# wangrui2025/GDKVM

Hardware: AMD Instinct MI355X
Metric: frames/sec (GDKVM forward + argmax mask), EchoNet 112x112x32 clips (higher is better)
Workload: dtype bf16; 1 GPU; BASELINE.json configs[1]: EchoNet-Dynamic 112x112x32 bf16 inference, batch=16 per GPU; clips_per_gpu=16, frames_per_clip=32, image=112x112, heads=1, key_dim=64, rule=delta_sequential, world_size=1, ranks_seen=1

## Files before the change

gdkvm_amd/csrc/conv_dispatch.hip:

```cpp
#include "gdkvm_common.hpp"

int gdkvm_conv3x3_c64_launch(const void* x, const void* w, const float* bias, const void* residual, void* y, int N, int H, int W,
                             int relu, int packed, hipStream_t st);
int gdkvm_conv3x3_tile_launch(const void* x, const void* x2, int C1, const void* w, const float* bias, const void* residual, void* y,
                              int N, int C, int H, int W, int K, int relu, int variant, int packed, hipStream_t st);
int gdkvm_conv_igemm_launch(const void* x, const void* wpacked, const float* bias, const void* residual, void* y,
                            int N, int C, int H, int W, int K, int R, int S, int stride, int pad, int relu,
                            const void* w2packed, const float* bias2, void* y2, hipStream_t st);

extern "C" int gdkvm_conv_bias_act(const void* x, const void* w, const float* bias, const void* residual, void* y,
                                   int N, int C, int H, int W, int K, int R, int S, int stride, int pad, int relu, int kernel,
                                   int io_dtype, void* stream)
{
    if (io_dtype != GDKVM_BF16) return gdkvm_fail(GDKVM_ERR_DTYPE, "conv_bias_act: only bf16 is implemented");
    if (N < 0 || C <= 0 || H <= 0 || W <= 0 || K <= 0 || R <= 0 || S <= 0 || stride <= 0 || pad < 0 || C % 8 || K % 8
        || H + 2 * pad < R || W + 2 * pad < S)
        return gdkvm_fail(GDKVM_ERR_SHAPE, "conv_bias_act: N=%d C=%d H=%d W=%d K=%d %dx%d stride %d pad %d (C, K multiples of 8)",
                          N, C, H, W, K, R, S, stride, pad);
    const bool packed = kernel & GDKVM_CONV_PACKED_WEIGHTS;
    kernel &= ~GDKVM_CONV_PACKED_WEIGHTS;
    if (kernel != 0 && (kernel < 4 || kernel > 11)) return gdkvm_fail(GDKVM_ERR_ARG, "conv_bias_act: kernel=%d (0 = by shape, 4, 5, 6..8, 9, 10, 11)", kernel);
    if (kernel == 9) {
        if (!packed) return gdkvm_fail(GDKVM_ERR_ARG, "conv_bias_act: kernel 9 reads the gdkvm_conv_igemm_pack_weights copy of the weights (flag %d)", GDKVM_CONV_PACKED_WEIGHTS);
        if (C % 32 || K % 128) return gdkvm_fail(GDKVM_ERR_SHAPE, "conv_bias_act: kernel 9 needs C a multiple of 32 and K of 128 (C=%d K=%d)", C, K);
        if (N == 0) return GDKVM_OK;
        if (!x || !w || !bias || !y) return gdkvm_fail(GDKVM_ERR_ARG, "conv_bias_act: null pointer");
        if (!gdkvm_aligned16(x) || !gdkvm_aligned16(w) || !gdkvm_aligned16(y) || !gdkvm_aligned16(bias) || (residual && !gdkvm_aligned16(residual)))
            return gdkvm_fail(GDKVM_ERR_ARG, "conv_bias_act: pointers must be 16-byte aligned");
        if (int rc = gdkvm_check_device()) return rc;
        if (gdkvm_conv_igemm_launch(x, w, bias, residual, y, N, C, H, W, K, R, S, stride, pad, relu, nullptr, nullptr, nullptr, static_cast<hipStream_t>(stream)))
            return gdkvm_fail(GDKVM_ERR_SHAPE, "conv_bias_act: N=%d C=%d H=%d W=%d K=%d %dx%d stride %d pad %d is too large for 32-bit offsets", N, C, H, W, K, R, S, stride, pad);
        GDKVM_LAUNCH_CHECK("conv_igemm_kernel");
        return GDKVM_OK;
    }
    if (packed && (C % 64 || K % 16))
        return gdkvm_fail(GDKVM_ERR_ARG, "conv_bias_act: packed weights need C a multiple of 64 and K of 16 (C=%d K=%d)", C, K);
    if (!(R == 3 && S == 3 && stride == 1 && pad == 1))
        return gdkvm_fail(GDKVM_ERR_SHAPE, "conv_bias_act: %dx%d stride %d pad %d is not served by the 3x3 / 1 / 1 kernels: kernel 9 (the "
                                           "implicit-GEMM kernel, packed weights) or the framework convolution + gdkvm_bias_act", R, S, stride, pad);
    if (N == 0) return GDKVM_OK;
    if (!x || !w || !bias || !y) return gdkvm_fail(GDKVM_ERR_ARG, "conv_bias_act: null pointer");
    if (!gdkvm_aligned16(x) || !gdkvm_aligned16(w) || !gdkvm_aligned16(y) || !gdkvm_aligned16(bias) || (residual && !gdkvm_aligned16(residual)))
        return gdkvm_fail(GDKVM_ERR_ARG, "conv_bias_act: pointers must be 16-byte aligned");
    if ((size_t)N * H * W * C >= (1ull << 31) || (size_t)N * H * W * K >= (1ull << 31))
        return gdkvm_fail(GDKVM_ERR_SHAPE, "conv_bias_act: tensor too large for 32-bit offsets");
    if (int rc = gdkvm_check_device()) return rc;
    hipStream_t st = static_cast<hipStream_t>(stream);
    const bool c64 = C == 64 && K == 64;
    if (kernel == 4 && !c64) return gdkvm_fail(GDKVM_ERR_SHAPE, "conv_bias_act: kernel 4 serves 64 -> 64 channels only (C=%d K=%d)", C, K);
    if (kernel == 4 || (kernel == 0 && c64)) {
        if (gdkvm_conv3x3_c64_launch(x, w, bias, residual, y, N, H, W, relu, packed ? 1 : 0, st)) return gdkvm_fail(GDKVM_ERR_SHAPE, "conv_bias_act: too many tiles");
        GDKVM_LAUNCH_CHECK("conv3x3_c64_kernel");
        return GDKVM_OK;
    }
    if (gdkvm_conv3x3_tile_launch(x, nullptr, 0, w, bias, residual, y, N, C, H, W, K, relu, kernel >= 10 ? kernel - 6 : (kernel >= 6 ? kernel - 5 : 0), packed ? 1 : 0, st))
        return gdkvm_fail(GDKVM_ERR_SHAPE, "conv_bias_act: C=%d K=%d %dx%d is not served by the hand-written kernels (C a multiple of 64, K of "
                                           "16, rows of at most 64 pixels): use the framework convolution + gdkvm_bias_act", C, K, H, W);
    GDKVM_LAUNCH_CHECK("conv3x3_tile_kernel");
    return GDKVM_OK;
}

extern "C" int gdkvm_conv_cat_bias_act(const void* x1, const void* x2, const void* w, const float* bias, const void* residual, void* y,
                                       int N, int C1, int C2, int H, int W, int K, int relu, int kernel, int io_dtype, void* stream)
{
    if (io_dtype != GDKVM_BF16) return gdkvm_fail(GDKVM_ERR_DTYPE, "conv_cat_bias_act: only bf16 is implemented");
    const bool packed = kernel & GDKVM_CONV_PACKED_WEIGHTS;
    kernel &= ~GDKVM_CONV_PACKED_WEIGHTS;
    if (kernel != 0 && (kernel < 5 || kernel > 11 || kernel == 9)) return gdkvm_fail(GDKVM_ERR_ARG, "conv_cat_bias_act: kernel=%d (0, 5..8, 10, 11)", kernel);
    if (N < 0 || C1 <= 0 || C2 <= 0 || C1 % 64 || C2 % 64 || H <= 0 || W <= 0 || K <= 0 || K % 16)
        return gdkvm_fail(GDKVM_ERR_SHAPE, "conv_cat_bias_act: N=%d C1=%d C2=%d H=%d W=%d K=%d (C1, C2 multiples of 64, K of 16)", N, C1, C2, H, W, K);
    if (N == 0) return GDKVM_OK;
    if (!x1 || !x2 || !w || !bias || !y) return gdkvm_fail(GDKVM_ERR_ARG, "conv_cat_bias_act: null pointer");
    if (!gdkvm_aligned16(x1) || !gdkvm_aligned16(x2) || !gdkvm_aligned16(w) || !gdkvm_aligned16(y) || !gdkvm_aligned16(bias) || (residual && !gdkvm_aligned16(residual)))
        return gdkvm_fail(GDKVM_ERR_ARG, "conv_cat_bias_act: pointers must be 16-byte aligned");
    if ((size_t)N * H * W * (C1 + C2) >= (1ull << 31) || (size_t)N * H * W * K >= (1ull << 31))
        return gdkvm_fail(GDKVM_ERR_SHAPE, "conv_cat_bias_act: tensor too large for 32-bit offsets");
    if (int rc = gdkvm_check_device()) return rc;
    if (gdkvm_conv3x3_tile_launch(x1, x2, C1, w, bias, residual, y, N, C1 + C2, H, W, K, relu, kernel >= 10 ? kernel - 6 : (kernel >= 6 ? kernel - 5 : 0), packed ? 1 : 0,
                                  static_cast<hipStream_t>(stream)))
        return gdkvm_fail(GDKVM_ERR_SHAPE, "conv_cat_bias_act: %dx%d is not served (rows of at most 64 pixels)", H, W);
    GDKVM_LAUNCH_CHECK("conv3x3_tile_kernel");
    return GDKVM_OK;
}

extern "C" int gdkvm_conv_down_bias_act(const void* x, const void* w, const float* bias, void* y, int relu,
                                        const void* w_down, const float* bias_down, void* y_down,
                                        int N, int C, int H, int W, int K, int R, int S, int stride, int pad, int io_dtype, void* stream)
{
    if (io_dtype != GDKVM_BF16) return gdkvm_fail(GDKVM_ERR_DTYPE, "conv_down_bias_act: only bf16 is implemented");
    if (N < 0 || C <= 0 || H <= 0 || W <= 0 || K <= 0 || R <= 0 || S != R || !(R & 1) || stride <= 0 || pad != R / 2 || C % 32 || K % 128)
        return gdkvm_fail(GDKVM_ERR_SHAPE, "conv_down_bias_act: N=%d C=%d H=%d W=%d K=%d %dx%d stride %d pad %d (odd square window, pad = R/2, "
                                           "C a multiple of 32, K of 128)", N, C, H, W, K, R, S, stride, pad);
    if (N == 0) return GDKVM_OK;
    if (!x || !w || !bias || !y || !w_down || !y_down) return gdkvm_fail(GDKVM_ERR_ARG, "conv_down_bias_act: null pointer");
    const void* ptrs[] = {x, w, bias, y, w_down, y_down};
    for (const void* p : ptrs) if (!gdkvm_aligned16(p)) return gdkvm_fail(GDKVM_ERR_ARG, "conv_down_bias_act: pointers must be 16-byte aligned");
    if (bias_down && !gdkvm_aligned16(bias_down)) return gdkvm_fail(GDKVM_ERR_ARG, "conv_down_bias_act: pointers must be 16-byte aligned");
    if (int rc = gdkvm_check_device()) return rc;
    if (gdkvm_conv_igemm_launch(x, w, bias, nullptr, y, N, C, H, W, K, R, S, stride, pad, relu, w_down, bias_down, y_down, static_cast<hipStream_t>(stream)))
        return gdkvm_fail(GDKVM_ERR_SHAPE, "conv_down_bias_act: tensor too large for 32-bit offsets");
    GDKVM_LAUNCH_CHECK("conv_igemm_kernel");
    return GDKVM_OK;
}
```

Measured before the change: 676,100 frames/s.

## Add persistent pipelined stride-2 3x3 conv kernel with fused downsample branch

Adds a dedicated kernel for 3x3 stride-2 convolutions fused with a 1x1 downsample projection. It runs a persistent grid sized to twice the CU count, stages input tiles into LDS through buffer-load-to-LDS DMA with a three-deep ring, and prefetches packed weights into registers so that loads overlap the MFMA work. conv_down_bias_act now routes to it when the shape qualifies and falls back to the implicit-GEMM kernel otherwise. The aim is to hide memory latency and cut launch and tail costs of the generic implicit-GEMM path, at the price of much hand-scheduled inline assembly and complex waitcnt logic that is hard to verify.

```diff
diff --git a/gdkvm_amd/csrc/conv_dispatch.hip b/gdkvm_amd/csrc/conv_dispatch.hip
--- a/gdkvm_amd/csrc/conv_dispatch.hip
+++ b/gdkvm_amd/csrc/conv_dispatch.hip
@@ -7,6 +7,8 @@
 int gdkvm_conv_igemm_launch(const void* x, const void* wpacked, const float* bias, const void* residual, void* y,
                             int N, int C, int H, int W, int K, int R, int S, int stride, int pad, int relu,
                             const void* w2packed, const float* bias2, void* y2, hipStream_t st);
+int gdkvm_conv_s2_block_launch(const void* x, const void* wpacked, const float* bias, void* y, int relu, const void* w2packed, const float* bias2, void* y2,
+                               int N, int C, int H, int W, int K, hipStream_t st);
 
 extern "C" int gdkvm_conv_bias_act(const void* x, const void* w, const float* bias, const void* residual, void* y,
                                    int N, int C, int H, int W, int K, int R, int S, int stride, int pad, int relu, int kernel,
@@ -97,6 +99,14 @@
     for (const void* p : ptrs) if (!gdkvm_aligned16(p)) return gdkvm_fail(GDKVM_ERR_ARG, "conv_down_bias_act: pointers must be 16-byte aligned");
     if (bias_down && !gdkvm_aligned16(bias_down)) return gdkvm_fail(GDKVM_ERR_ARG, "conv_down_bias_act: pointers must be 16-byte aligned");
     if (int rc = gdkvm_check_device()) return rc;
+    if (R == 3 && stride == 2) {
+        const int rc = gdkvm_conv_s2_block_launch(x, w, bias, y, relu, w_down, bias_down, y_down, N, C, H, W, K, static_cast<hipStream_t>(stream));
+        if (rc < 0) return gdkvm_fail(GDKVM_ERR_LAUNCH, "conv_down_bias_act: the device query for the block kernel's grid failed");
+        if (rc == 0) {
+            GDKVM_LAUNCH_CHECK("conv_s2_block_kernel");
+            return GDKVM_OK;
+        }
+    }
     if (gdkvm_conv_igemm_launch(x, w, bias, nullptr, y, N, C, H, W, K, R, S, stride, pad, relu, w_down, bias_down, y_down, static_cast<hipStream_t>(stream)))
         return gdkvm_fail(GDKVM_ERR_SHAPE, "conv_down_bias_act: tensor too large for 32-bit offsets");
     GDKVM_LAUNCH_CHECK("conv_igemm_kernel");
diff --git a/gdkvm_amd/csrc/conv_s2_block.hip b/gdkvm_amd/csrc/conv_s2_block.hip
--- /dev/null
+++ b/gdkvm_amd/csrc/conv_s2_block.hip
@@ -0,0 +1,251 @@
+#include <atomic>
+#include <type_traits>
+
+#include "gdkvm_common.hpp"
+
+namespace {
+
+constexpr int SB_TM = 128, SB_TN = 128;
+constexpr int SB_PIX = 160;
+constexpr int SB_SLOTS = SB_PIX / 16;
+constexpr int SB_BUF = SB_TM * SB_PIX;
+constexpr int SB_RING = 3;
+constexpr int SB_PP = SB_BUF / 1024 / 4;
+constexpr int SB_MT = SB_TM / 16, SB_NTW = 2;
+constexpr unsigned SB_DEAD = 0x80000000u;
+constexpr size_t SB_LDS = (size_t)SB_RING * SB_BUF + 2 * SB_TN * sizeof(float);
+
+struct S2Args {
+    const bf16_t* x; const bf16_t* w; const bf16_t* w2; const float* bias; const float* bias2; bf16_t* y; bf16_t* y2;
+    int H, W, C, K, Wo, HWo, M, relu;
+    int spt, ntiles;
+    unsigned xbytes;
+    int step_q, step_r;
+    float inv_hwo, inv_wo;
+};
+
+__device__ __forceinline__ int sb_div(int n, float inv) { return (int)(((float)n + 0.5f) * inv); }
+
+template <int I, int E, class F>
+__device__ __forceinline__ void sb_static_for(F&& f)
+{
+    if constexpr (I < E) {
+        f(std::integral_constant<int, I>{});
+        sb_static_for<I + 1, E>(f);
+    }
+}
+
+__global__ __launch_bounds__(256, 2) void conv_s2_block_kernel(S2Args a)
+{
+    extern __shared__ __attribute__((aligned(16))) unsigned char sb_lds[];
+    const int tid = threadIdx.x, lane = tid & 63, li = lane & 15, g = lane >> 4;
+    const int w = __builtin_amdgcn_readfirstlane(tid >> 6);
+    const int n0 = blockIdx.y * SB_TN;
+    const int gx = (int)gridDim.x;
+    const int nsteps = 9 * a.spt;
+
+    float* const s_bias = reinterpret_cast<float*>(sb_lds + SB_RING * SB_BUF);
+    if (tid < SB_TN) {
+        s_bias[tid] = a.bias[n0 + tid];
+        s_bias[SB_TN + tid] = a.bias2 ? a.bias2[n0 + tid] : 0.f;
+    }
+
+    const __amdgpu_buffer_rsrc_t rsrc = __builtin_amdgcn_make_buffer_rsrc(const_cast<bf16_t*>(a.x), 0, (int)a.xbytes, 0x00020000);
+    const unsigned lds0 = (unsigned)reinterpret_cast<uintptr_t>(sb_lds);
+    unsigned g_off[SB_PP], topm = 0, leftm = 0;
+    int tile_d = blockIdx.x, m0_d = tile_d * SB_TM;
+    int f0 = m0_d / a.HWo, rem0 = m0_d - f0 * a.HWo;
+    auto set_geo = [&]() __attribute__((always_inline)) {
+        topm = 0; leftm = 0;
+        const int last = a.M - 1 - m0_d;
+#pragma unroll
+        for (int u = 0; u < SB_PP; ++u) {
+            const int d = 64 * (w + 4 * u) + lane, pix = sb_div(d, 1.0f / SB_SLOTS), c = d - SB_SLOTS * pix;
+            const int loc = rem0 + min(pix, last);
+            const int fl = sb_div(loc, a.inv_hwo), r = loc - fl * a.HWo, yo = sb_div(r, a.inv_wo), xo = r - yo * a.Wo;
+            const int src = (((f0 + fl) * a.H + 2 * yo - 1) * a.W + 2 * xo - 1) * a.C + 8 * c;
+            const bool live = c < 8;
+            g_off[u] = live ? (unsigned)(src * 2) : SB_DEAD;
+            topm |= live && yo == 0 ? 1u << u : 0u;
+            leftm |= live && xo == 0 ? 1u << u : 0u;
+        }
+    };
+    int dr = 0, dsx = 0, dsub = 0;
+    auto dma = [&](int buf) __attribute__((always_inline)) {
+        const unsigned ts = (unsigned)(((dr * a.W + dsx) * a.C + dsub * 64) * 2);
+        const unsigned kill = (dr == 0 ? topm : 0u) | (dsx == 0 ? leftm : 0u);
+        const unsigned dst0 = lds0 + buf * SB_BUF + 1024 * w;
+#pragma unroll
+        for (int u = 0; u < SB_PP; ++u) {
+            const unsigned voff = (kill >> u) & 1u ? SB_DEAD : g_off[u] + ts;
+            __builtin_amdgcn_raw_ptr_buffer_load_lds(rsrc, reinterpret_cast<__attribute__((address_space(3))) void*>(static_cast<uintptr_t>(dst0 + 4096 * u)), 16,
+                                                     (int)voff, 0, 0, 0);
+        }
+        if (++dsub == a.spt) { dsub = 0; if (++dsx == 3) { dsx = 0; ++dr; } }
+    };
+    auto next_tile = [&]() __attribute__((always_inline)) {
+        dr = 0;
+        if (tile_d + gx < a.ntiles) {
+            tile_d += gx; m0_d += gx * SB_TM;
+            f0 += a.step_q; rem0 += a.step_r;
+            if (rem0 >= a.HWo) { rem0 -= a.HWo; ++f0; }
+            set_geo();
+        }
+    };
+
+    struct WK { bf16x8 f[SB_NTW]; };
+    struct WB { bf16x8 f[2 * SB_NTW]; };
+    const bf16_t* const wbase = a.w + (size_t)(n0 / 16 + SB_NTW * w) * (size_t)(2 * nsteps) * 512;
+    const bf16_t* const bbase = a.w2 + (size_t)(n0 / 16 + SB_NTW * w) * (size_t)(2 * a.spt) * 512;
+    const unsigned wv0 = (unsigned)lane * 16u, wv1 = wv0 + (unsigned)(2 * nsteps) * 1024u, bv1 = wv0 + (unsigned)(2 * a.spt) * 1024u;
+    WK wr[SB_RING];
+    WB br;
+    int wpos = 0;
+    auto kload = [&](WK& o) __attribute__((always_inline)) {
+        const bf16_t* const base = wbase + (size_t)wpos * 512;
+        asm volatile("global_load_dwordx4 %0, %1, %2" : "=&v"(o.f[0]) : "v"(wv0), "s"(base) : "memory");
+        asm volatile("global_load_dwordx4 %0, %1, %2" : "=&v"(o.f[1]) : "v"(wv1), "s"(base) : "memory");
+        if (++wpos == 2 * nsteps) wpos = 0;
+    };
+    auto bload = [&](int i) __attribute__((always_inline)) {
+        const bf16_t* const base = bbase + (size_t)i * 1024;
+        asm volatile("global_load_dwordx4 %0, %1, %2" : "=&v"(br.f[0]) : "v"(wv0), "s"(base) : "memory");
+        asm volatile("global_load_dwordx4 %0, %1, %2" : "=&v"(br.f[1]) : "v"(bv1), "s"(base) : "memory");
+        asm volatile("global_load_dwordx4 %0, %1, %2 offset:1024" : "=&v"(br.f[2]) : "v"(wv0), "s"(base) : "memory");
+        asm volatile("global_load_dwordx4 %0, %1, %2 offset:1024" : "=&v"(br.f[3]) : "v"(bv1), "s"(base) : "memory");
+    };
+
+    set_geo();
+    __builtin_amdgcn_sched_barrier(0);
+    dma(0); kload(wr[0]); dma(1); kload(wr[1]); kload(wr[2]);
+    asm volatile("s_waitcnt vmcnt(%0)" :: "n"(SB_PP + 3 * SB_NTW) : "memory");
+#pragma unroll
+    for (int q = 0; q < 4; ++q) br.f[q] = bf16x8{};
+
+    const unsigned char* const xrd = sb_lds + li * SB_PIX + 16 * g;
+    const int c_lo = 4 * a.spt;
+
+    for (int tile = blockIdx.x; tile < a.ntiles; tile += gx) {
+        f32x4 acc[SB_MT][SB_NTW], acc2[SB_MT][SB_NTW];
+#pragma unroll
+        for (int mt = 0; mt < SB_MT; ++mt)
+#pragma unroll
+            for (int nt = 0; nt < SB_NTW; ++nt) { acc[mt][nt] = f32x4{0.f, 0.f, 0.f, 0.f}; acc2[mt][nt] = f32x4{0.f, 0.f, 0.f, 0.f}; }
+        int l = 0;
+        auto step = [&](auto jc) __attribute__((always_inline)) {
+            constexpr int j = decltype(jc)::value, sA = (2 * j) % SB_RING, sB = (2 * j + 1) % SB_RING;
+            asm volatile("s_waitcnt vmcnt(%0) lgkmcnt(0)\n\ts_barrier" :: "n"(4 * SB_NTW + SB_PP) : "memory");
+            dma((j + 2) % SB_RING);
+            const unsigned char* const xb = xrd + j * SB_BUF;
+            auto readg = [&](bf16x8 (&xg)[4], int h) __attribute__((always_inline)) {
+#pragma unroll
+                for (int q = 0; q < 4; ++q) xg[q] = *reinterpret_cast<const bf16x8*>(xb + (4 * (h & 1) + q) * 16 * SB_PIX + 64 * (h >> 1));
+            };
+            const bool centre = (unsigned)(l - c_lo) < (unsigned)a.spt;
+            bf16x8 xg[2][4];
+            readg(xg[0], 0);
+            asm volatile("s_waitcnt vmcnt(%2)" : "+v"(wr[sA].f[0]), "+v"(wr[sA].f[1]) : "n"(2 * SB_NTW + 2 * SB_PP) : "memory");
+            if (centre) asm volatile("s_waitcnt vmcnt(%4)" : "+v"(br.f[0]), "+v"(br.f[1]), "+v"(br.f[2]), "+v"(br.f[3]) : "n"(SB_NTW + SB_PP) : "memory");
+            sb_static_for<0, 4>([&](auto hc) {
+                constexpr int h = decltype(hc)::value, sb = h >> 1, half = h & 1, set = sb ? sB : sA;
+                if constexpr (h == 2) asm volatile("s_waitcnt vmcnt(%2)" : "+v"(wr[sB].f[0]), "+v"(wr[sB].f[1]) : "n"(2 * SB_NTW + SB_PP) : "memory");
+                if constexpr (h < 3) readg(xg[(h + 1) & 1], h + 1);
+#pragma unroll
+                for (int q = 0; q < 4; ++q)
+#pragma unroll
+                    for (int nt = 0; nt < SB_NTW; ++nt)
+                        acc[4 * half + q][nt] = __builtin_amdgcn_mfma_f32_16x16x32_bf16(wr[set].f[nt], xg[h & 1][q], acc[4 * half + q][nt], 0, 0, 0);
+                if (centre) {
+#pragma unroll
+                    for (int q = 0; q < 4; ++q)
+#pragma unroll
+                        for (int nt = 0; nt < SB_NTW; ++nt)
+                            acc2[4 * half + q][nt] = __builtin_amdgcn_mfma_f32_16x16x32_bf16(br.f[2 * sb + nt], xg[h & 1][q], acc2[4 * half + q][nt], 0, 0, 0);
+                }
+                __builtin_amdgcn_sched_barrier(0);
+                if constexpr (h == 1) { kload(wr[sA]); __builtin_amdgcn_sched_barrier(0); }
+            });
+            ++l;
+            if ((unsigned)(l - c_lo) < (unsigned)a.spt) bload(l - c_lo);
+            kload(wr[sB]);
+            __builtin_amdgcn_sched_barrier(0);
+        };
+#pragma unroll 1
+        for (int trip = 0; trip < 3 * a.spt; ++trip) {
+            step(std::integral_constant<int, 0>{});
+            if (trip == 3 * a.spt - 1) next_tile();
+            step(std::integral_constant<int, 1>{});
+            step(std::integral_constant<int, 2>{});
+        }
+
+        {
+            const int m0 = tile * SB_TM;
+            const float lo = a.relu ? 0.f : -INFINITY;
+            auto pk4 = [](const f32x4& v) { return make_uint2((unsigned)f32_to_bf16(v[0]) | ((unsigned)f32_to_bf16(v[1]) << 16), (unsigned)f32_to_bf16(v[2]) | ((unsigned)f32_to_bf16(v[3]) << 16)); };
+#pragma unroll
+            for (int nt = 0; nt < SB_NTW; ++nt) {
+                const int cw = 16 * SB_NTW * w + 16 * nt + 4 * g;
+                const f32x4 b4 = *reinterpret_cast<const f32x4*>(s_bias + cw), d4 = *reinterpret_cast<const f32x4*>(s_bias + SB_TN + cw);
+#pragma unroll
+                for (int mt = 0; mt < SB_MT; ++mt) {
+                    const int p = m0 + 16 * mt + li;
+                    f32x4 v = acc[mt][nt] + b4, v2 = acc2[mt][nt] + d4;
+#pragma unroll
+                    for (int r = 0; r < 4; ++r) { v[r] = fmaxf(v[r], lo); v2[r] = fmaxf(v2[r], -INFINITY); }
+                    const uint2 o1 = pk4(v), o2 = pk4(v2);
+                    const size_t o = (size_t)p * a.K + n0 + cw;
+                    bf16_t* const yp = a.y + o;
+                    bf16_t* const yp2 = a.y2 + o;
+                    if (p < a.M) asm volatile("global_store_dwordx2 %0, %1, off\n\tglobal_store_dwordx2 %2, %3, off\n\ts_nop 1" :: "v"(yp), "v"(o1), "v"(yp2), "v"(o2) : "memory");
+                }
+            }
+        }
+    }
+    asm volatile("s_waitcnt vmcnt(0)" ::: "memory");
+}
+
+}
+
+struct S2Plan { int ok, Ho, Wo, M, ntiles, gx, gy, step_q, step_r; };
+static S2Plan s2_plan(int N, int C, int H, int W, int K, int cus)
+{
+    S2Plan p{};
+    if (N < 1 || H < 2 || W < 2 || (H & 1) || (W & 1) || C < 64 || C % 64 || K < SB_TN || K % SB_TN || cus < 1) return p;
+    p.Ho = H / 2; p.Wo = W / 2;
+    const long long M = (long long)N * p.Ho * p.Wo;
+    if ((long long)N * H * W * C * 2 >= 0x7fffffffLL || M * K * 2 >= 0x7fffffffLL || (long long)p.Ho * p.Wo + SB_TM >= (1 << 21) || 9 * (C / 64) > 32767) return p;
+    p.M = (int)M;
+    p.ntiles = (int)((M + SB_TM - 1) / SB_TM);
+    p.gy = K / SB_TN;
+    int per = 2 * cus / p.gy; if (per < 1) per = 1;
+    p.gx = p.ntiles < per ? p.ntiles : per;
+    const long long stride = (long long)p.gx * SB_TM;
+    p.step_q = (int)(stride / (p.Ho * p.Wo)); p.step_r = (int)(stride % (p.Ho * p.Wo));
+    p.ok = 1;
+    return p;
+}
+
+int gdkvm_conv_s2_block_launch(const void* x, const void* wpacked, const float* bias, void* y, int relu, const void* w2packed, const float* bias2, void* y2,
+                               int N, int C, int H, int W, int K, hipStream_t st)
+{
+    static std::atomic<int> cus_of[64];
+    int dev = 0;
+    if (hipGetDevice(&dev) != hipSuccess || dev < 0) return -1;
+    int cus = dev < 64 ? cus_of[dev].load(std::memory_order_relaxed) : 0;
+    if (cus == 0) {
+        if (hipDeviceGetAttribute(&cus, hipDeviceAttributeMultiprocessorCount, dev) != hipSuccess || cus < 1) return -1;
+        if (dev < 64) cus_of[dev].store(cus, std::memory_order_relaxed);
+    }
+    const S2Plan p = s2_plan(N, C, H, W, K, cus);
+    if (!p.ok || !w2packed || !y2 || !bias) return 1;
+    S2Args a{};
+    a.x = static_cast<const bf16_t*>(x); a.w = static_cast<const bf16_t*>(wpacked); a.w2 = static_cast<const bf16_t*>(w2packed);
+    a.bias = bias; a.bias2 = bias2; a.y = static_cast<bf16_t*>(y); a.y2 = static_cast<bf16_t*>(y2);
+    a.H = H; a.W = W; a.C = C; a.K = K; a.Wo = p.Wo; a.HWo = p.Ho * p.Wo; a.M = p.M; a.relu = relu;
+    a.spt = C / 64; a.ntiles = p.ntiles;
+    a.xbytes = (unsigned)((long long)N * H * W * C * 2);
+    a.step_q = p.step_q; a.step_r = p.step_r;
+    a.inv_hwo = 1.0f / (float)a.HWo; a.inv_wo = 1.0f / (float)a.Wo;
+    hipLaunchKernelGGL(conv_s2_block_kernel, dim3((unsigned)p.gx, (unsigned)p.gy), dim3(256), SB_LDS, st, a);
+    return 0;
+}
```

Measured after the change: 678,500 frames/s (median of 5 runs). Within noise of the previous version (+0.4%).
